# PKU-DAIR/Hetu-Galvatron

Measured on NVIDIA H100. Metric: tokens/sec Llama-3.2-1B-shaped ZeRO-2 training step at 1/2/4/8 H100 vs ref CPU, higher is better.
Workload: dtype bf16

## Files before the change

### hetu-galvatron_b200/csrc/bg_gemm.cu

```cuda
#include <stdlib.h>

#include "bg_ctx.cuh"

using namespace bg;

namespace {

constexpr int BLOCK_M = 128, BLOCK_N = 128, BLOCK_K = 64, WGMMA_K = 16;
constexpr int kStages = 5;
constexpr int kABytes = BLOCK_M * BLOCK_K * 2, kBBytes = BLOCK_N * BLOCK_K * 2, kStageBytes = kABytes + kBBytes;
constexpr int kStoreCols = 64;
constexpr int kStoreBytes = BLOCK_M * kStoreCols * 2;
constexpr int kNumStoreBufs = 2;
constexpr int kSmemBytes = kStages * kStageBytes + kNumStoreBufs * kStoreBytes + 1024  + 256 ;
constexpr int kEpiThreads = 256, kThreads = kEpiThreads + 32;
constexpr int kProducerWarp = kEpiThreads / 32;
constexpr int kMaxRegs = 136;
constexpr int kWgOffset = 8192;
constexpr int kGroupM = 16;
static_assert(kSmemBytes <= 227 * 1024, "H100: at most 227 KiB of shared memory per block");
static_assert(kThreads * kMaxRegs + 3 * 128 * 64 <= 65536, "a GEMM CTA and three slim collective CTAs share an SM's registers");
static_assert(kSmemBytes + 1024 + 3 * 1024 <= 228 * 1024, "a GEMM CTA and three slim collective CTAs share an SM's shared memory");

enum Layout { kTN = 0, kNN = 1, kNT = 2 };

__device__ __forceinline__ uint32_t smem_u32(const void* p) { return (uint32_t)__cvta_generic_to_shared(p); }

__device__ __forceinline__ void mbar_init(uint32_t bar, uint32_t count) {
    asm volatile("mbarrier.init.shared::cta.b64 [%0], %1;" ::"r"(bar), "r"(count));
}
__device__ __forceinline__ void mbar_wait(uint32_t bar, uint32_t parity) {
    asm volatile(
        "{\n\t.reg .pred p;\n\t"
        "WAIT_%=:\n\t"
        "mbarrier.try_wait.parity.shared::cta.b64 p, [%0], %1;\n\t"
        "@p bra DONE_%=;\n\t"
        "bra WAIT_%=;\n\t"
        "DONE_%=:\n\t}" ::"r"(bar), "r"(parity) : "memory");
}
__device__ __forceinline__ void mbar_arrive(uint32_t bar) {
    asm volatile("mbarrier.arrive.shared::cta.b64 _, [%0];" ::"r"(bar) : "memory");
}
__device__ __forceinline__ void mbar_expect_tx(uint32_t bar, uint32_t bytes) {
    asm volatile("mbarrier.arrive.expect_tx.shared::cta.b64 _, [%0], %1;" ::"r"(bar), "r"(bytes) : "memory");
}
__device__ __forceinline__ void tma_load_2d(uint32_t dst, const CUtensorMap* map, uint32_t bar, int c0, int c1) {
    asm volatile("cp.async.bulk.tensor.2d.shared::cluster.global.mbarrier::complete_tx::bytes [%0], [%1, {%3, %4}], [%2];"
                 ::"r"(dst), "l"(map), "r"(bar), "r"(c0), "r"(c1) : "memory");
}
__device__ __forceinline__ void tma_store_2d(const CUtensorMap* map, uint32_t src, int c0, int c1) {
    asm volatile("cp.async.bulk.tensor.2d.global.shared::cta.bulk_group [%0, {%2, %3}], [%1];"
                 ::"l"(map), "r"(src), "r"(c0), "r"(c1) : "memory");
}
__device__ __forceinline__ void tma_store_commit() { asm volatile("cp.async.bulk.commit_group;" ::: "memory"); }
template <int N>
__device__ __forceinline__ void tma_store_wait_read() { asm volatile("cp.async.bulk.wait_group.read %0;" ::"n"(N) : "memory"); }
template <int N>
__device__ __forceinline__ void tma_store_wait_all() { asm volatile("cp.async.bulk.wait_group %0;" ::"n"(N) : "memory"); }
__device__ __forceinline__ void fence_proxy_async() { asm volatile("fence.proxy.async.shared::cta;" ::: "memory"); }
__device__ __forceinline__ void epi_bar_sync() { asm volatile("bar.sync 1, %0;" ::"n"(kEpiThreads) : "memory"); }
__device__ __forceinline__ bool elect_one() {
    uint32_t pred;
    asm volatile("{\n\t.reg .pred p;\n\telect.sync _|p, 0xffffffff;\n\tselp.u32 %0, 1, 0, p;\n\t}" : "=r"(pred));
    return pred != 0;
}

__device__ __forceinline__ void wgmma_fence() { asm volatile("wgmma.fence.sync.aligned;" ::: "memory"); }
__device__ __forceinline__ void wgmma_commit() { asm volatile("wgmma.commit_group.sync.aligned;" ::: "memory"); }
template <int N>
__device__ __forceinline__ void wgmma_wait() { asm volatile("wgmma.wait_group.sync.aligned %0;" ::"n"(N) : "memory"); }
__device__ __forceinline__ void fence_acc(float* d) {
#pragma unroll
    for (int i = 0; i < BLOCK_N / 2; ++i) asm volatile("" : "+f"(d[i])::"memory");
}

template <int kTransA, int kTransB>
__device__ __forceinline__ void wgmma_m64n128(float* d, uint64_t desc_a, uint64_t desc_b, uint32_t accumulate) {
    asm volatile(
        "{\n\t.reg .pred p;\n\t"
        "setp.ne.b32 p, %66, 0;\n\t"
        "wgmma.mma_async.sync.aligned.m64n128k16.f32.bf16.bf16 "
        "{%0, %1, %2, %3, %4, %5, %6, %7, %8, %9, %10, %11, %12, %13, %14, %15, "
        "%16, %17, %18, %19, %20, %21, %22, %23, %24, %25, %26, %27, %28, %29, %30, %31, "
        "%32, %33, %34, %35, %36, %37, %38, %39, %40, %41, %42, %43, %44, %45, %46, %47, "
        "%48, %49, %50, %51, %52, %53, %54, %55, %56, %57, %58, %59, %60, %61, %62, %63}, "
        "%64, %65, p, 1, 1, %67, %68;\n\t}"
        : "+f"(d[0]), "+f"(d[1]), "+f"(d[2]), "+f"(d[3]), "+f"(d[4]), "+f"(d[5]), "+f"(d[6]), "+f"(d[7]),
          "+f"(d[8]), "+f"(d[9]), "+f"(d[10]), "+f"(d[11]), "+f"(d[12]), "+f"(d[13]), "+f"(d[14]), "+f"(d[15]),
          "+f"(d[16]), "+f"(d[17]), "+f"(d[18]), "+f"(d[19]), "+f"(d[20]), "+f"(d[21]), "+f"(d[22]), "+f"(d[23]),
          "+f"(d[24]), "+f"(d[25]), "+f"(d[26]), "+f"(d[27]), "+f"(d[28]), "+f"(d[29]), "+f"(d[30]), "+f"(d[31]),
          "+f"(d[32]), "+f"(d[33]), "+f"(d[34]), "+f"(d[35]), "+f"(d[36]), "+f"(d[37]), "+f"(d[38]), "+f"(d[39]),
          "+f"(d[40]), "+f"(d[41]), "+f"(d[42]), "+f"(d[43]), "+f"(d[44]), "+f"(d[45]), "+f"(d[46]), "+f"(d[47]),
          "+f"(d[48]), "+f"(d[49]), "+f"(d[50]), "+f"(d[51]), "+f"(d[52]), "+f"(d[53]), "+f"(d[54]), "+f"(d[55]),
          "+f"(d[56]), "+f"(d[57]), "+f"(d[58]), "+f"(d[59]), "+f"(d[60]), "+f"(d[61]), "+f"(d[62]), "+f"(d[63])
        : "l"(desc_a), "l"(desc_b), "r"(accumulate), "n"(kTransA), "n"(kTransB));
}

__device__ __forceinline__ uint64_t make_smem_desc(uint32_t smem_addr, uint32_t lbo_bytes, uint32_t sbo_bytes) {
    uint64_t d = 0;
    d |= (uint64_t)((smem_addr >> 4) & 0x3fff);
    d |= (uint64_t)((lbo_bytes >> 4) & 0x3fff) << 16;
    d |= (uint64_t)((sbo_bytes >> 4) & 0x3fff) << 32;
    d |= (uint64_t)1 << 62;
    return d;
}

struct TileCoord { int m, n; };
enum { kPlain = 0, kScatterMode = 1, kGatherMode = 2 };

template <int kMode>
struct FuseParams {};

template <>
struct FuseParams<kPlain> {
    int group_m;
};

__device__ __forceinline__ TileCoord tile_of_virtual(int t, int m_blocks, int n_blocks, int group_m) {
    const int per_group = group_m * n_blocks;
    const int g = t / per_group, first_m = g * group_m;
    const int rows = min(group_m, m_blocks - first_m);
    const int r = t - g * per_group;
    return {first_m + r % rows, r / rows};
}

template <>
struct FuseParams<kScatterMode> {
    CUtensorMap dst[BG_MAX_PEERS];
    uint32_t* flags[BG_MAX_PEERS];
    int p, me, rows_per_rank;
};

template <>
struct FuseParams<kGatherMode> {
    CUtensorMap a_local;
    const uint32_t* flags;
    uint32_t target;
    int p, me, blocks_per_rank;
    unsigned long long timeout_ns;
    int* err;
};

template <int kMode>
__device__ __forceinline__ int map_m(int mv, int m_blocks, const FuseParams<kMode>& fp) {
    if constexpr (kMode == kScatterMode) {
        int m = mv + ((fp.me + 1) % fp.p) * (fp.rows_per_rank / BLOCK_M);
        return m >= m_blocks ? m - m_blocks : m;
    } else if constexpr (kMode == kGatherMode) {
        const int c = mv / fp.p, k = mv - c * fp.p;
        int slot = fp.me + k; if (slot >= fp.p) slot -= fp.p;
        return slot * fp.blocks_per_rank + c;
    } else {
        return mv;
    }
}
template <int kMode>
__device__ __forceinline__ TileCoord tile_of(int t, int m_blocks, int n_blocks, const FuseParams<kMode>& fp) {
    int group_m = kGroupM;
    if constexpr (kMode == kPlain) group_m = fp.group_m;
    TileCoord tc = tile_of_virtual(t, m_blocks, n_blocks, group_m);
    tc.m = map_m<kMode>(tc.m, m_blocks, fp);
    return tc;
}

template <int kLayout, int kMode = kPlain>
__global__ void __maxnreg__(kMaxRegs) gemm_bf16_kernel(const __grid_constant__ CUtensorMap map_a,
                                                                const __grid_constant__ CUtensorMap map_b,
                                                                const __grid_constant__ CUtensorMap map_c,
                                                                const __nv_bfloat16* __restrict__ c_old, int M, int N, int K,
                                                                int accumulate,
                                                                const __grid_constant__ FuseParams<kMode> sp) {
    constexpr bool kScatter = kMode == kScatterMode, kGather = kMode == kGatherMode;
    constexpr bool kAMn = kLayout == kNT, kBMn = kLayout != kTN;
    extern __shared__ uint8_t smem_raw[];
    uint8_t* smem = reinterpret_cast<uint8_t*>((reinterpret_cast<uintptr_t>(smem_raw) + 1023) & ~uintptr_t(1023));
    uint8_t* smem_store = smem + kStages * kStageBytes;
    uint64_t* bars = reinterpret_cast<uint64_t*>(smem_store + kNumStoreBufs * kStoreBytes);
    uint64_t* full_bar = bars;
    uint64_t* empty_bar = bars + kStages;

    const int warp = threadIdx.x >> 5, lane = threadIdx.x & 31;
    const int m_blocks = (M + BLOCK_M - 1) / BLOCK_M, n_blocks = (N + BLOCK_N - 1) / BLOCK_N;
    const int num_tiles = m_blocks * n_blocks, k_blocks = (K + BLOCK_K - 1) / BLOCK_K;

    if constexpr (kScatter) {
        asm volatile("griddepcontrol.launch_dependents;" ::: "memory");
    }
    if (warp == kProducerWarp && lane == 0) {
        asm volatile("prefetch.tensormap [%0];" ::"l"(&map_a) : "memory");
        asm volatile("prefetch.tensormap [%0];" ::"l"(&map_b) : "memory");
        asm volatile("prefetch.tensormap [%0];" ::"l"(&map_c) : "memory");
        for (int i = 0; i < kStages; ++i) { mbar_init(smem_u32(full_bar + i), 1); mbar_init(smem_u32(empty_bar + i), kEpiThreads / 32); }
        asm volatile("fence.mbarrier_init.release.cluster;" ::: "memory");
    }
    __syncthreads();

    if (warp == kProducerWarp) {
        if (elect_one()) {
            int stage = 0; uint32_t phase = 0;
            for (int t = blockIdx.x; t < num_tiles; t += gridDim.x) {
                const TileCoord tc = tile_of<kMode>(t, m_blocks, n_blocks, sp);
                const CUtensorMap* amap = &map_a;
                int a_row = tc.m * BLOCK_M;
                if constexpr (kGather) {
                    const int slot = tc.m / sp.blocks_per_rank, c = tc.m - slot * sp.blocks_per_rank;
                    if (slot == sp.me) {
                        amap = &sp.a_local; a_row = c * BLOCK_M;
                    } else {
                        const uint32_t* f = sp.flags + slot * sp.blocks_per_rank + c;
                        unsigned long long t0 = 0; unsigned spins = 0;
                        while (true) {
                            uint32_t v;
                            asm volatile("ld.acquire.sys.global.u32 %0, [%1];" : "=r"(v) : "l"(f) : "memory");
                            if (v >= sp.target) break;
                            if ((++spins & 0x3ff) == 0) {
                                unsigned long long now = gtimer();
                                if (t0 == 0) t0 = now;
                                else if (now - t0 > sp.timeout_ns) {
                                    if (atomicCAS(sp.err + 1, 0, 4) == 0) { sp.err[2] = (int)blockIdx.x; sp.err[3] = tc.m; sp.err[4] = (int)v; sp.err[5] = (int)sp.target; sp.err[6] = slot; }
                                    *sp.err = BG_ETIMEOUT; __threadfence_system(); __trap();
                                }
                            }
                        }
                        asm volatile("fence.proxy.async.global;" ::: "memory");
                    }
                }
                for (int kb = 0; kb < k_blocks; ++kb) {
                    mbar_wait(smem_u32(empty_bar + stage), phase ^ 1);
                    const uint32_t bar = smem_u32(full_bar + stage);
                    const uint32_t sa = smem_u32(smem + stage * kStageBytes), sb = sa + kABytes;
                    mbar_expect_tx(bar, kStageBytes);
                    if (kAMn) {
#pragma unroll
                        for (int j = 0; j < BLOCK_M / 64; ++j) tma_load_2d(sa + j * (BLOCK_K * 128), &map_a, bar, tc.m * BLOCK_M + j * 64, kb * BLOCK_K);
                    } else {
                        tma_load_2d(sa, amap, bar, kb * BLOCK_K, a_row);
                    }
                    if (kBMn) {
#pragma unroll
                        for (int j = 0; j < BLOCK_N / 64; ++j) tma_load_2d(sb + j * (BLOCK_K * 128), &map_b, bar, tc.n * BLOCK_N + j * 64, kb * BLOCK_K);
                    } else {
                        tma_load_2d(sb, &map_b, bar, kb * BLOCK_K, tc.n * BLOCK_N);
                    }
                    if (++stage == kStages) { stage = 0; phase ^= 1; }
                }
            }
        }
    } else {
        const int wg = warp >> 2;
        const int frag_row = wg * 64 + (warp & 3) * 16 + (lane >> 2);
        const int frag_col = (lane & 3) * 2;
        const bool issuer = threadIdx.x == 0;
        constexpr uint32_t a_lbo = kAMn ? BLOCK_K * 128 : 0, b_lbo = kBMn ? BLOCK_K * 128 : 0;
        constexpr uint32_t a_kstep = kAMn ? WGMMA_K * 128 : WGMMA_K * 2, b_kstep = kBMn ? WGMMA_K * 128 : WGMMA_K * 2;
        float acc[BLOCK_N / 2];
#pragma unroll
        for (int i = 0; i < BLOCK_N / 2; ++i) acc[i] = 0.f;
        int stage = 0; uint32_t phase = 0;
        int buf = 0;
        uint32_t* prev_flag = nullptr;
        for (int t = blockIdx.x; t < num_tiles; t += gridDim.x) {
            const TileCoord tc = tile_of<kMode>(t, m_blocks, n_blocks, sp);
            int prev_stage = 0;
            for (int kb = 0; kb < k_blocks; ++kb) {
                mbar_wait(smem_u32(full_bar + stage), phase);
                const uint32_t sa = smem_u32(smem + stage * kStageBytes) + wg * kWgOffset;
                const uint32_t sb = smem_u32(smem + stage * kStageBytes) + kABytes;
                wgmma_fence();
#pragma unroll
                for (int k = 0; k < BLOCK_K / WGMMA_K; ++k) {
                    const uint64_t da = make_smem_desc(sa + k * a_kstep, a_lbo, 1024);
                    const uint64_t db = make_smem_desc(sb + k * b_kstep, b_lbo, 1024);
                    wgmma_m64n128<kAMn ? 1 : 0, kBMn ? 1 : 0>(acc, da, db, (kb | k) != 0);
                }
                wgmma_commit();
                wgmma_wait<1>();
                if (kb > 0 && lane == 0) mbar_arrive(smem_u32(empty_bar + prev_stage));
                prev_stage = stage;
                if (++stage == kStages) { stage = 0; phase ^= 1; }
            }
            wgmma_wait<0>();
            fence_acc(acc);
            if (lane == 0) mbar_arrive(smem_u32(empty_bar + prev_stage));
#pragma unroll
            for (int c = 0; c < BLOCK_N / kStoreCols; ++c) {
                const int n0 = tc.n * BLOCK_N + c * kStoreCols;
                if (n0 >= N) break;
                float* v = acc + c * (kStoreCols / 2);
                if (accumulate) {
#pragma unroll
                    for (int h = 0; h < 2; ++h) {
                        const long long grow = (long long)tc.m * BLOCK_M + frag_row + 8 * h;
                        if (grow < M) {
#pragma unroll
                            for (int j = 0; j < 8; ++j) {
                                if (n0 + j * 8 < N) {
                                    const float2 o = bf2_to_f2(*reinterpret_cast<const uint32_t*>(c_old + grow * N + n0 + j * 8 + frag_col));
                                    v[j * 4 + 2 * h] += o.x;
                                    v[j * 4 + 2 * h + 1] += o.y;
                                }
                            }
                        }
                    }
                }
                if (issuer) tma_store_wait_read<kNumStoreBufs - 1>();
                epi_bar_sync();
                uint8_t* sbuf = smem_store + buf * kStoreBytes;
#pragma unroll
                for (int h = 0; h < 2; ++h) {
                    const int row = frag_row + 8 * h;
#pragma unroll
                    for (int j = 0; j < 8; ++j)
                        *reinterpret_cast<uint32_t*>(sbuf + row * 128 + ((j ^ (row & 7)) << 4) + frag_col * 2) =
                            f2_to_bf2(v[j * 4 + 2 * h], v[j * 4 + 2 * h + 1]);
                }
                fence_proxy_async();
                epi_bar_sync();
                if (issuer) {
                    if constexpr (kScatter) {
                        const int row0 = tc.m * BLOCK_M, owner = row0 / sp.rows_per_rank;
                        tma_store_2d(&sp.dst[owner], smem_u32(sbuf), n0, sp.me * sp.rows_per_rank + (row0 - owner * sp.rows_per_rank));
                    } else {
                        tma_store_2d(&map_c, smem_u32(sbuf), n0, tc.m * BLOCK_M);
                    }
                    tma_store_commit();
                }
                buf ^= 1;
            }
            if constexpr (kScatter) {
                if (issuer) {
                    if (prev_flag != nullptr) {
                        asm volatile("cp.async.bulk.wait_group %0;" ::"n"(BLOCK_N / kStoreCols) : "memory");
                        __threadfence_system();
                        asm volatile("red.release.sys.global.add.u32 [%0], 1;" ::"l"(prev_flag) : "memory");
                    }
                    const int row0 = tc.m * BLOCK_M, owner = row0 / sp.rows_per_rank;
                    prev_flag = sp.flags[owner] + ((row0 - owner * sp.rows_per_rank) / BLOCK_M) * n_blocks + tc.n;
                }
            }
        }
        if (issuer) {
            tma_store_wait_all<0>();
            if constexpr (kScatter) {
                if (prev_flag != nullptr) {
                    __threadfence_system();
                    asm volatile("red.release.sys.global.add.u32 [%0], 1;" ::"l"(prev_flag) : "memory");
                }
            }
        }
    }
}

typedef CUresult (*EncodeTiledFn)(CUtensorMap*, CUtensorMapDataType, cuuint32_t, void*, const cuuint64_t*, const cuuint64_t*,
                                  const cuuint32_t*, const cuuint32_t*, CUtensorMapInterleave, CUtensorMapSwizzle,
                                  CUtensorMapL2promotion, CUtensorMapFloatOOBfill);

EncodeTiledFn encode_fn() {
    static EncodeTiledFn fn = nullptr;
    static std::once_flag once;
    std::call_once(once, [] {
        void* p = nullptr;
        cudaDriverEntryPointQueryResult q;
        if (cudaGetDriverEntryPoint("cuTensorMapEncodeTiled", &p, cudaEnableDefault, &q) == cudaSuccess && q == cudaDriverEntryPointSuccess)
            fn = (EncodeTiledFn)p;
    });
    return fn;
}

int make_map(CUtensorMap* map, const void* ptr, long long rows, long long cols, int box_cols, int box_rows) {
    EncodeTiledFn fn = encode_fn();
    if (!fn) return fail(BG_ECUDA, "cuTensorMapEncodeTiled entry point not available");
    cuuint64_t dims[2] = {(cuuint64_t)cols, (cuuint64_t)rows};
    cuuint64_t strides[1] = {(cuuint64_t)cols * 2};
    cuuint32_t box[2] = {(cuuint32_t)box_cols, (cuuint32_t)box_rows};
    cuuint32_t estr[2] = {1, 1};
    CUresult r = fn(map, CU_TENSOR_MAP_DATA_TYPE_BFLOAT16, 2, const_cast<void*>(ptr), dims, strides, box, estr,
                    CU_TENSOR_MAP_INTERLEAVE_NONE, CU_TENSOR_MAP_SWIZZLE_128B, CU_TENSOR_MAP_L2_PROMOTION_L2_256B,
                    CU_TENSOR_MAP_FLOAT_OOB_FILL_NONE);
    if (r == CUDA_ERROR_INVALID_CONTEXT) {
        cudaFree(0);
        r = fn(map, CU_TENSOR_MAP_DATA_TYPE_BFLOAT16, 2, const_cast<void*>(ptr), dims, strides, box, estr,
               CU_TENSOR_MAP_INTERLEAVE_NONE, CU_TENSOR_MAP_SWIZZLE_128B, CU_TENSOR_MAP_L2_PROMOTION_L2_256B,
               CU_TENSOR_MAP_FLOAT_OOB_FILL_NONE);
    }
    if (r != CUDA_SUCCESS) return fail(BG_ECUDA, "cuTensorMapEncodeTiled failed (%d) rows=%lld cols=%lld", (int)r, rows, cols);
    return BG_OK;
}

int g_num_sms = 0;

}

int bg_preload_gemm();

static int gemm_setup() {
    if (g_num_sms == 0) {
        int dev = 0;
        BG_CUDA(cudaGetDevice(&dev));
        int sms = 0;
        BG_CUDA(cudaDeviceGetAttribute(&sms, cudaDevAttrMultiProcessorCount, dev));
#define BG_SMEM(K) BG_CUDA(cudaFuncSetAttribute(K, cudaFuncAttributeMaxDynamicSharedMemorySize, kSmemBytes))
        BG_SMEM(gemm_bf16_kernel<kTN>); BG_SMEM(gemm_bf16_kernel<kNN>); BG_SMEM(gemm_bf16_kernel<kNT>);
        BG_SMEM((gemm_bf16_kernel<kTN, kScatterMode>)); BG_SMEM((gemm_bf16_kernel<kNN, kScatterMode>)); BG_SMEM((gemm_bf16_kernel<kNT, kScatterMode>));
        BG_SMEM((gemm_bf16_kernel<kTN, kGatherMode>)); BG_SMEM((gemm_bf16_kernel<kNN, kGatherMode>));
#undef BG_SMEM
        g_num_sms = sms;
    }
    return BG_OK;
}



static int make_ab_maps(CUtensorMap* ma, CUtensorMap* mb, const void* a, const void* b, long long m, long long n, long long k, int layout) {
    int rc = layout == kNT ? make_map(ma, a, k, m, 64, BLOCK_K) : make_map(ma, a, m, k, BLOCK_K, BLOCK_M);
    if (rc) return rc;
    return layout == kTN ? make_map(mb, b, n, k, BLOCK_K, BLOCK_N) : make_map(mb, b, k, n, 64, BLOCK_K);
}

static int gemm_launch(const void* a, const void* b, void* c, const void* addend, long long m, long long n, long long k, int layout, void* stream);

extern "C" int bg_gemm_bf16(const void* a, const void* b, void* c, long long m, long long n, long long k, int layout,
                            int accumulate, void* stream) {
    return gemm_launch(a, b, c, accumulate ? c : nullptr, m, n, k, layout, stream);
}

extern "C" int bg_gemm_bf16_add(const void* a, const void* b, void* c, const void* addend, long long m, long long n, long long k,
                                int layout, void* stream) {
    if (addend == nullptr || (uintptr_t)addend % 16) return fail(BG_EINVAL, "bg_gemm_bf16_add: addend must be a 16-B aligned [M][N] bf16 tensor");
    return gemm_launch(a, b, c, addend, m, n, k, layout, stream);
}

static int gemm_launch(const void* a, const void* b, void* c, const void* addend, long long m, long long n, long long k, int layout, void* stream) {
    const int accumulate = addend != nullptr;
    if (layout < 0 || layout > 2) return fail(BG_EINVAL, "bg_gemm_bf16: layout %d", layout);
    if (m <= 0 || n <= 0 || k <= 0 || m % 8 || n % 8 || k % 8)
        return fail(BG_EINVAL, "bg_gemm_bf16: m,n,k (%lld,%lld,%lld) must be positive multiples of 8", m, n, k);
    if (((uintptr_t)a | (uintptr_t)b | (uintptr_t)c) % 16) return fail(BG_EINVAL, "bg_gemm_bf16: pointers must be 16-B aligned");
    CUtensorMap ma, mb, mc;
    int rc = make_ab_maps(&ma, &mb, a, b, m, n, k, layout);
    if (rc) return rc;
    rc = make_map(&mc, c, m, n, kStoreCols, BLOCK_M);
    if (rc) return rc;
    rc = gemm_setup();
    if (rc) return rc;
    const long long n_blocks = (n + BLOCK_N - 1) / BLOCK_N, tiles = ((m + BLOCK_M - 1) / BLOCK_M) * n_blocks;
    const int grid = (int)(tiles < g_num_sms ? tiles : g_num_sms);
    cudaStream_t st = (cudaStream_t)stream;
    const __nv_bfloat16* c_old = (const __nv_bfloat16*)addend;
    FuseParams<kPlain> plain;
    plain.group_m = n_blocks <= 32 ? 2 : 8;
    if (layout == kTN) gemm_bf16_kernel<kTN><<<grid, kThreads, kSmemBytes, st>>>(ma, mb, mc, c_old, (int)m, (int)n, (int)k, accumulate, plain);
    else if (layout == kNN) gemm_bf16_kernel<kNN><<<grid, kThreads, kSmemBytes, st>>>(ma, mb, mc, c_old, (int)m, (int)n, (int)k, accumulate, plain);
    else gemm_bf16_kernel<kNT><<<grid, kThreads, kSmemBytes, st>>>(ma, mb, mc, c_old, (int)m, (int)n, (int)k, accumulate, plain);
    BG_CHECK_LAUNCH();
    return BG_OK;
}

namespace {

struct Bcast {
    char* out[BG_MAX_PEERS];
    char* mc;
    int on;
};

__device__ __forceinline__ void mm_st_16g(void* mc, const uint4& v) {
    asm volatile("multimem.st.relaxed.sys.global.v4.f32 [%0], {%1,%2,%3,%4};" ::"l"(mc), "f"(__uint_as_float(v.x)),
                 "f"(__uint_as_float(v.y)), "f"(__uint_as_float(v.z)), "f"(__uint_as_float(v.w)) : "memory");
}

__global__ void __launch_bounds__(128, 8) tile_reduce_kernel(const __nv_bfloat16* __restrict__ partial, uint32_t* __restrict__ flags,
                                                          __nv_bfloat16* __restrict__ out, int p, int me, int rows_per_rank, int N,
                                                          int n_blocks, int local_tiles, const __grid_constant__ Bcast bc,
                                                          unsigned long long timeout_ns, int* err) {
    for (int lt = blockIdx.x; lt < local_tiles; lt += gridDim.x) {
        if (threadIdx.x == 0) {
            unsigned long long t0 = 0;
            unsigned spins = 0;
            while (true) {
                uint32_t v;
                asm volatile("ld.acquire.sys.global.u32 %0, [%1];" : "=r"(v) : "l"(flags + lt) : "memory");
                if (v >= (uint32_t)p) break;
                if ((++spins & 0x3ff) == 0) {
                    unsigned long long now = gtimer();
                    if (t0 == 0) t0 = now;
                    else if (now - t0 > timeout_ns / 2) {
                        if (atomicCAS(err + 1, 0, 3) == 0) { err[2] = (int)blockIdx.x; err[3] = lt; err[4] = (int)v; err[5] = p; err[6] = local_tiles; }
                        *err = BG_ETIMEOUT; __threadfence_system(); __trap();
                    }
                }
            }
        }
        __syncthreads();
        const int mb = lt / n_blocks, nb = lt % n_blocks;
        const int row0 = mb * BLOCK_M, col0 = nb * BLOCK_N;
        const int cols = min(BLOCK_N, N - col0), rows = min(BLOCK_M, rows_per_rank - row0);
        const int vec_per_row = cols / 8;
        for (int i = threadIdx.x; i < rows * vec_per_row; i += blockDim.x) {
            const int r = i / vec_per_row, c = i - r * vec_per_row;
            const size_t off = (size_t)(row0 + r) * N + col0 + c * 8;
            uint4 in[BG_MAX_PEERS];
#pragma unroll
            for (int src = 0; src < BG_MAX_PEERS; ++src)
                if (src < p) in[src] = ld16_stream(partial + (size_t)src * rows_per_rank * N + off);
            float acc[8];
#pragma unroll
            for (int e = 0; e < 8; ++e) acc[e] = 0.f;
#pragma unroll
            for (int src = 0; src < BG_MAX_PEERS; ++src)
                if (src < p) {
                    float f[8];
                    unpack8(in[src], f);
#pragma unroll
                    for (int e = 0; e < 8; ++e) acc[e] += f[e];
                }
            const uint4 o = pack8(acc);
            if (bc.on) {
                const size_t goff = ((size_t)me * rows_per_rank * N + off) * 2;
                if (bc.mc != nullptr) {
                    mm_st_16g(bc.mc + goff, o);
                } else {
                    for (int k = 0; k < p; ++k) {
                        int q = me + k; if (q >= p) q -= p;
                        st16(bc.out[q] + goff, o);
                    }
                }
            } else {
                st16(out + off, o);
            }
        }
        __syncthreads();
        if (threadIdx.x == 0) flags[lt] = 0;
    }
    asm volatile("griddepcontrol.wait;" ::: "memory");
}

}

int bg_gemm_scatter_launch(const void* a, const void* b, long long m, long long n, long long k, int layout, int p, int me,
                           void* const* partial_ptrs, uint32_t* const* flag_ptrs, void* out, void* const* bcast_ptrs, char* bcast_mc,
                           unsigned long long timeout_ns, int* err_dev, cudaStream_t st) {
    if (layout < 0 || layout > 2) return fail(BG_EINVAL, "bg_gemm_reduce_scatter: layout %d", layout);
    if (m <= 0 || n <= 0 || k <= 0 || n % 8 || k % 8) return fail(BG_EINVAL, "bg_gemm_reduce_scatter: bad dims");
    if (m % ((long long)p * BLOCK_M)) return fail(BG_EINVAL, "bg_gemm_reduce_scatter: M=%lld must be a multiple of p*%d", m, BLOCK_M);
    const int rows_per_rank = (int)(m / p);
    CUtensorMap ma, mb;
    int rc = make_ab_maps(&ma, &mb, a, b, m, n, k, layout);
    if (rc) return rc;
    FuseParams<kScatterMode> sp;
    sp.p = p; sp.me = me; sp.rows_per_rank = rows_per_rank;
    for (int i = 0; i < BG_MAX_PEERS; ++i) {
        sp.flags[i] = i < p ? flag_ptrs[i] : nullptr;
        if (i < p) { rc = make_map(&sp.dst[i], partial_ptrs[i], (long long)p * rows_per_rank, n, kStoreCols, BLOCK_M); if (rc) return rc; }
        else sp.dst[i] = sp.dst[0];
    }
    rc = gemm_setup();
    if (rc) return rc;
    const int m_blocks = (int)((m + BLOCK_M - 1) / BLOCK_M), n_blocks = (int)((n + BLOCK_N - 1) / BLOCK_N);
    const long long tiles = (long long)m_blocks * n_blocks;
    const int grid = (int)(tiles < g_num_sms ? tiles : g_num_sms);
    const int local_tiles = (rows_per_rank / BLOCK_M) * n_blocks;
    const CUtensorMap& mc_unused = sp.dst[0];
    if (layout == kTN) gemm_bf16_kernel<kTN, kScatterMode><<<grid, kThreads, kSmemBytes, st>>>(ma, mb, mc_unused, nullptr, (int)m, (int)n, (int)k, 0, sp);
    else if (layout == kNN) gemm_bf16_kernel<kNN, kScatterMode><<<grid, kThreads, kSmemBytes, st>>>(ma, mb, mc_unused, nullptr, (int)m, (int)n, (int)k, 0, sp);
    else gemm_bf16_kernel<kNT, kScatterMode><<<grid, kThreads, kSmemBytes, st>>>(ma, mb, mc_unused, nullptr, (int)m, (int)n, (int)k, 0, sp);
    BG_CHECK_LAUNCH();
    const int rgrid = local_tiles < g_num_sms ? local_tiles : g_num_sms;
    Bcast bc = {};
    if (bcast_ptrs != nullptr) {
        bc.on = 1; bc.mc = bcast_mc;
        for (int i = 0; i < p; ++i) bc.out[i] = (char*)bcast_ptrs[i];
    }
    cudaLaunchConfig_t cfg = {};
    cfg.gridDim = dim3((unsigned)rgrid); cfg.blockDim = dim3(128);
    cudaLaunchAttribute attr[1];
    attr[0].id = cudaLaunchAttributeProgrammaticStreamSerialization;
    attr[0].val.programmaticStreamSerializationAllowed = 1;
    static const bool no_pdl = getenv("HGB_NO_PDL") != nullptr;
    cfg.attrs = attr; cfg.numAttrs = no_pdl ? 0 : 1;
    BG_CUDA(cudaLaunchKernelEx(&cfg, tile_reduce_kernel, (const __nv_bfloat16*)partial_ptrs[me], (uint32_t*)flag_ptrs[me],
                               (__nv_bfloat16*)out, p, me, rows_per_rank, (int)n, n_blocks, local_tiles, bc, timeout_ns, err_dev));
    bg::g_launches.fetch_add(1, std::memory_order_relaxed);
    return BG_OK;
}

int bg_gemm_gather_launch(const void* a_local, const void* a_staged, const void* b, void* c, long long m, long long n, long long k,
                          int layout, int p, int me, const uint32_t* flags, uint32_t target, unsigned long long timeout_ns, int* err_dev,
                          cudaStream_t st) {
    if (layout != kTN && layout != kNN) return fail(BG_EINVAL, "bg_all_gather_gemm: layout %d", layout);
    if (((uintptr_t)a_local | (uintptr_t)a_staged | (uintptr_t)b | (uintptr_t)c) % 16) return fail(BG_EINVAL, "bg_all_gather_gemm: pointers must be 16-B aligned");
    CUtensorMap ma, mb, mc;
    int rc = make_ab_maps(&ma, &mb, a_staged, b, m, n, k, layout);
    if (rc) return rc;
    rc = make_map(&mc, c, m, n, kStoreCols, BLOCK_M);
    if (rc) return rc;
    FuseParams<kGatherMode> gp;
    rc = make_map(&gp.a_local, a_local, m / p, k, BLOCK_K, BLOCK_M);
    if (rc) return rc;
    gp.flags = flags; gp.target = target; gp.p = p; gp.me = me; gp.blocks_per_rank = (int)(m / p / BLOCK_M);
    gp.timeout_ns = timeout_ns; gp.err = err_dev;
    rc = gemm_setup();
    if (rc) return rc;
    const long long tiles = (m / BLOCK_M) * ((n + BLOCK_N - 1) / BLOCK_N);
    const int grid = (int)(tiles < g_num_sms ? tiles : g_num_sms);
    if (layout == kTN) gemm_bf16_kernel<kTN, kGatherMode><<<grid, kThreads, kSmemBytes, st>>>(ma, mb, mc, nullptr, (int)m, (int)n, (int)k, 0, gp);
    else gemm_bf16_kernel<kNN, kGatherMode><<<grid, kThreads, kSmemBytes, st>>>(ma, mb, mc, nullptr, (int)m, (int)n, (int)k, 0, gp);
    BG_CHECK_LAUNCH();
    return BG_OK;
}

int bg_preload_gemm() {
    int rc = gemm_setup();
    if (rc) return rc;
    cudaFuncAttributes attr;
    BG_CUDA(cudaFuncGetAttributes(&attr, reinterpret_cast<const void*>(&tile_reduce_kernel)));
    return BG_OK;
}
```

Before: 39510.

## Prefetch GEMM addend via TMA and split epilogue per warpgroup

For plain-mode GEMMs, the addend tile is now loaded by TMA into the store buffers partway through the K loop, instead of being read with scattered global loads in the epilogue. Each warpgroup then writes its own 64-row half of both column chunks, syncs on a per-warpgroup named barrier, and issues its own TMA stores, so the two halves no longer wait on each other. The goal is to hide addend load latency and cut epilogue synchronisation. The cost is that the store buffers are no longer double-buffered across chunks: the code must wait for earlier stores to drain before the next tile's epilogue or C load.

Result: no change. 39230 (median of 6 runs) (-0.7%).

```diff
diff --git a/hetu-galvatron_b200/csrc/bg_gemm.cu b/hetu-galvatron_b200/csrc/bg_gemm.cu
--- a/hetu-galvatron_b200/csrc/bg_gemm.cu
+++ b/hetu-galvatron_b200/csrc/bg_gemm.cu
@@ -17,6 +17,9 @@
 constexpr int kProducerWarp = kEpiThreads / 32;
 constexpr int kMaxRegs = 136;
 constexpr int kWgOffset = 8192;
+constexpr int kWgRows = 64;
+constexpr int kWgStoreBytes = kWgRows * kStoreCols * 2;
+constexpr int kCLoadKb = 2;
 constexpr int kGroupM = 16;
 static_assert(kSmemBytes <= 227 * 1024, "H100: at most 227 KiB of shared memory per block");
 static_assert(kThreads * kMaxRegs + 3 * 128 * 64 <= 65536, "a GEMM CTA and three slim collective CTAs share an SM's registers");
@@ -59,6 +62,10 @@
 __device__ __forceinline__ void tma_store_wait_all() { asm volatile("cp.async.bulk.wait_group %0;" ::"n"(N) : "memory"); }
 __device__ __forceinline__ void fence_proxy_async() { asm volatile("fence.proxy.async.shared::cta;" ::: "memory"); }
 __device__ __forceinline__ void epi_bar_sync() { asm volatile("bar.sync 1, %0;" ::"n"(kEpiThreads) : "memory"); }
+__device__ __forceinline__ void wg_bar_sync(int wg) {
+    if (wg == 0) asm volatile("bar.sync 2, 128;" ::: "memory");
+    else asm volatile("bar.sync 3, 128;" ::: "memory");
+}
 __device__ __forceinline__ bool elect_one() {
     uint32_t pred;
     asm volatile("{\n\t.reg .pred p;\n\telect.sync _|p, 0xffffffff;\n\tselp.u32 %0, 1, 0, p;\n\t}" : "=r"(pred));
@@ -114,6 +121,7 @@
 template <>
 struct FuseParams<kPlain> {
     int group_m;
+    CUtensorMap c_src;
 };
 
 __device__ __forceinline__ TileCoord tile_of_virtual(int t, int m_blocks, int n_blocks, int group_m) {
@@ -178,6 +186,7 @@
     uint64_t* bars = reinterpret_cast<uint64_t*>(smem_store + kNumStoreBufs * kStoreBytes);
     uint64_t* full_bar = bars;
     uint64_t* empty_bar = bars + kStages;
+    uint64_t* c_full = bars + 2 * kStages;
 
     const int warp = threadIdx.x >> 5, lane = threadIdx.x & 31;
     const int m_blocks = (M + BLOCK_M - 1) / BLOCK_M, n_blocks = (N + BLOCK_N - 1) / BLOCK_N;
@@ -191,6 +200,10 @@
         asm volatile("prefetch.tensormap [%0];" ::"l"(&map_b) : "memory");
         asm volatile("prefetch.tensormap [%0];" ::"l"(&map_c) : "memory");
         for (int i = 0; i < kStages; ++i) { mbar_init(smem_u32(full_bar + i), 1); mbar_init(smem_u32(empty_bar + i), kEpiThreads / 32); }
+        if constexpr (kMode == kPlain) {
+            if (accumulate) asm volatile("prefetch.tensormap [%0];" ::"l"(&sp.c_src) : "memory");
+            for (int i = 0; i < 2; ++i) mbar_init(smem_u32(c_full + i), 1);
+        }
         asm volatile("fence.mbarrier_init.release.cluster;" ::: "memory");
     }
     __syncthreads();
@@ -250,7 +263,9 @@
         const int wg = warp >> 2;
         const int frag_row = wg * 64 + (warp & 3) * 16 + (lane >> 2);
         const int frag_col = (lane & 3) * 2;
-        const bool issuer = threadIdx.x == 0;
+        const bool issuer = kMode == kPlain ? (threadIdx.x & 127) == 0 : threadIdx.x == 0;
+        const bool has_c = kMode == kPlain && accumulate;
+        uint32_t c_phase = 0;
         constexpr uint32_t a_lbo = kAMn ? BLOCK_K * 128 : 0, b_lbo = kBMn ? BLOCK_K * 128 : 0;
         constexpr uint32_t a_kstep = kAMn ? WGMMA_K * 128 : WGMMA_K * 2, b_kstep = kBMn ? WGMMA_K * 128 : WGMMA_K * 2;
         float acc[BLOCK_N / 2];
@@ -262,6 +277,7 @@
         for (int t = blockIdx.x; t < num_tiles; t += gridDim.x) {
             const TileCoord tc = tile_of<kMode>(t, m_blocks, n_blocks, sp);
             int prev_stage = 0;
+            const int n_chunks = tc.n * BLOCK_N + kStoreCols < N ? 2 : 1;
             for (int kb = 0; kb < k_blocks; ++kb) {
                 mbar_wait(smem_u32(full_bar + stage), phase);
                 const uint32_t sa = smem_u32(smem + stage * kStageBytes) + wg * kWgOffset;
@@ -274,6 +290,16 @@
                     wgmma_m64n128<kAMn ? 1 : 0, kBMn ? 1 : 0>(acc, da, db, (kb | k) != 0);
                 }
                 wgmma_commit();
+                if constexpr (kMode == kPlain) {
+                    if (has_c && issuer && kb == min(kCLoadKb, k_blocks - 1)) {
+                        tma_store_wait_read<0>();
+                        const uint32_t bar = smem_u32(c_full + wg);
+                        mbar_expect_tx(bar, n_chunks * kWgStoreBytes);
+                        for (int c = 0; c < n_chunks; ++c)
+                            tma_load_2d(smem_u32(smem_store + c * kStoreBytes + wg * kWgStoreBytes), &sp.c_src, bar,
+                                        tc.n * BLOCK_N + c * kStoreCols, tc.m * BLOCK_M + wg * kWgRows);
+                    }
+                }
                 wgmma_wait<1>();
                 if (kb > 0 && lane == 0) mbar_arrive(smem_u32(empty_bar + prev_stage));
                 prev_stage = stage;
@@ -282,50 +308,87 @@
             wgmma_wait<0>();
             fence_acc(acc);
             if (lane == 0) mbar_arrive(smem_u32(empty_bar + prev_stage));
-#pragma unroll
-            for (int c = 0; c < BLOCK_N / kStoreCols; ++c) {
-                const int n0 = tc.n * BLOCK_N + c * kStoreCols;
-                if (n0 >= N) break;
-                float* v = acc + c * (kStoreCols / 2);
-                if (accumulate) {
+            if constexpr (kMode == kPlain) {
+                if (!has_c && issuer) tma_store_wait_read<0>();
+                epi_bar_sync();
+                if (has_c) {
+                    mbar_wait(smem_u32(c_full + wg), c_phase);
+                    c_phase ^= 1;
+                }
+#pragma unroll
+                for (int c = 0; c < BLOCK_N / kStoreCols; ++c) {
+                    if (c >= n_chunks) break;
+                    float* v = acc + c * (kStoreCols / 2);
+                    uint8_t* sbuf = smem_store + c * kStoreBytes;
 #pragma unroll
                     for (int h = 0; h < 2; ++h) {
-                        const long long grow = (long long)tc.m * BLOCK_M + frag_row + 8 * h;
-                        if (grow < M) {
-#pragma unroll
-                            for (int j = 0; j < 8; ++j) {
-                                if (n0 + j * 8 < N) {
-                                    const float2 o = bf2_to_f2(*reinterpret_cast<const uint32_t*>(c_old + grow * N + n0 + j * 8 + frag_col));
-                                    v[j * 4 + 2 * h] += o.x;
-                                    v[j * 4 + 2 * h + 1] += o.y;
+                        const int row = frag_row + 8 * h;
+#pragma unroll
+                        for (int j = 0; j < 8; ++j) {
+                            uint32_t* p = reinterpret_cast<uint32_t*>(sbuf + row * 128 + ((j ^ (row & 7)) << 4) + frag_col * 2);
+                            if (has_c) {
+                                const float2 o = bf2_to_f2(*p);
+                                v[j * 4 + 2 * h] += o.x;
+                                v[j * 4 + 2 * h + 1] += o.y;
+                            }
+                            *p = f2_to_bf2(v[j * 4 + 2 * h], v[j * 4 + 2 * h + 1]);
+                        }
+                    }
+                }
+                fence_proxy_async();
+                wg_bar_sync(wg);
+                if (issuer) {
+                    for (int c = 0; c < n_chunks; ++c)
+                        tma_store_2d(&map_c, smem_u32(smem_store + c * kStoreBytes + wg * kWgStoreBytes),
+                                     tc.n * BLOCK_N + c * kStoreCols, tc.m * BLOCK_M + wg * kWgRows);
+                    tma_store_commit();
+                }
+            } else {
+#pragma unroll
+                for (int c = 0; c < BLOCK_N / kStoreCols; ++c) {
+                    const int n0 = tc.n * BLOCK_N + c * kStoreCols;
+                    if (n0 >= N) break;
+                    float* v = acc + c * (kStoreCols / 2);
+                    if (accumulate) {
+#pragma unroll
+                        for (int h = 0; h < 2; ++h) {
+                            const long long grow = (long long)tc.m * BLOCK_M + frag_row + 8 * h;
+                            if (grow < M) {
+#pragma unroll
+                                for (int j = 0; j < 8; ++j) {
+                                    if (n0 + j * 8 < N) {
+                                        const float2 o = bf2_to_f2(*reinterpret_cast<const uint32_t*>(c_old + grow * N + n0 + j * 8 + frag_col));
+                                        v[j * 4 + 2 * h] += o.x;
+                                        v[j * 4 + 2 * h + 1] += o.y;
+                                    }
                                 }
                             }
                         }
                     }
-                }
-                if (issuer) tma_store_wait_read<kNumStoreBufs - 1>();
-                epi_bar_sync();
-                uint8_t* sbuf = smem_store + buf * kStoreBytes;
-#pragma unroll
-                for (int h = 0; h < 2; ++h) {
-                    const int row = frag_row + 8 * h;
-#pragma unroll
-                    for (int j = 0; j < 8; ++j)
-                        *reinterpret_cast<uint32_t*>(sbuf + row * 128 + ((j ^ (row & 7)) << 4) + frag_col * 2) =
-                            f2_to_bf2(v[j * 4 + 2 * h], v[j * 4 + 2 * h + 1]);
-                }
-                fence_proxy_async();
-                epi_bar_sync();
-                if (issuer) {
-                    if constexpr (kScatter) {
-                        const int row0 = tc.m * BLOCK_M, owner = row0 / sp.rows_per_rank;
-                        tma_store_2d(&sp.dst[owner], smem_u32(sbuf), n0, sp.me * sp.rows_per_rank + (row0 - owner * sp.rows_per_rank));
-                    } else {
-                        tma_store_2d(&map_c, smem_u32(sbuf), n0, tc.m * BLOCK_M);
-                    }
-                    tma_store_commit();
-                }
-                buf ^= 1;
+                    if (issuer) tma_store_wait_read<kNumStoreBufs - 1>();
+                    epi_bar_sync();
+                    uint8_t* sbuf = smem_store + buf * kStoreBytes;
+#pragma unroll
+                    for (int h = 0; h < 2; ++h) {
+                        const int row = frag_row + 8 * h;
+#pragma unroll
+                        for (int j = 0; j < 8; ++j)
+                            *reinterpret_cast<uint32_t*>(sbuf + row * 128 + ((j ^ (row & 7)) << 4) + frag_col * 2) =
+                                f2_to_bf2(v[j * 4 + 2 * h], v[j * 4 + 2 * h + 1]);
+                    }
+                    fence_proxy_async();
+                    epi_bar_sync();
+                    if (issuer) {
+                        if constexpr (kScatter) {
+                            const int row0 = tc.m * BLOCK_M, owner = row0 / sp.rows_per_rank;
+                            tma_store_2d(&sp.dst[owner], smem_u32(sbuf), n0, sp.me * sp.rows_per_rank + (row0 - owner * sp.rows_per_rank));
+                        } else {
+                            tma_store_2d(&map_c, smem_u32(sbuf), n0, tc.m * BLOCK_M);
+                        }
+                        tma_store_commit();
+                    }
+                    buf ^= 1;
+                }
             }
             if constexpr (kScatter) {
                 if (issuer) {
@@ -436,18 +499,24 @@
     if (m <= 0 || n <= 0 || k <= 0 || m % 8 || n % 8 || k % 8)
         return fail(BG_EINVAL, "bg_gemm_bf16: m,n,k (%lld,%lld,%lld) must be positive multiples of 8", m, n, k);
     if (((uintptr_t)a | (uintptr_t)b | (uintptr_t)c) % 16) return fail(BG_EINVAL, "bg_gemm_bf16: pointers must be 16-B aligned");
+    FuseParams<kPlain> plain;
     CUtensorMap ma, mb, mc;
     int rc = make_ab_maps(&ma, &mb, a, b, m, n, k, layout);
     if (rc) return rc;
-    rc = make_map(&mc, c, m, n, kStoreCols, BLOCK_M);
-    if (rc) return rc;
+    rc = make_map(&mc, c, m, n, kStoreCols, kWgRows);
+    if (rc) return rc;
+    if (addend != nullptr) {
+        rc = make_map(&plain.c_src, addend, m, n, kStoreCols, kWgRows);
+        if (rc) return rc;
+    } else {
+        memset(&plain.c_src, 0, sizeof(plain.c_src));
+    }
     rc = gemm_setup();
     if (rc) return rc;
     const long long n_blocks = (n + BLOCK_N - 1) / BLOCK_N, tiles = ((m + BLOCK_M - 1) / BLOCK_M) * n_blocks;
     const int grid = (int)(tiles < g_num_sms ? tiles : g_num_sms);
     cudaStream_t st = (cudaStream_t)stream;
     const __nv_bfloat16* c_old = (const __nv_bfloat16*)addend;
-    FuseParams<kPlain> plain;
     plain.group_m = n_blocks <= 32 ? 2 : 8;
     if (layout == kTN) gemm_bf16_kernel<kTN><<<grid, kThreads, kSmemBytes, st>>>(ma, mb, mc, c_old, (int)m, (int)n, (int)k, accumulate, plain);
     else if (layout == kNN) gemm_bf16_kernel<kNN><<<grid, kThreads, kSmemBytes, st>>>(ma, mb, mc, c_old, (int)m, (int)n, (int)k, accumulate, plain);
```
